# iwa-shi/DC_VIC

Hardware: AMD Instinct MI355X
Metric: images/sec encode+decode @256x256 q=0 (higher is better)
Workload: dtype f32

## Files before the change

dc_vic_amd/csrc/conv.hip:

```cpp
#include "conv_common.h"

template <int MT, int NT, int WM, int WN, bool UPS>
__global__ __launch_bounds__(NTHREADS, (MT * NT >= 8) ? 2 : ((MT * NT >= 4) ? 3 : 4)) void conv_mfma_kernel(const ConvKArgs K) {
    constexpr int TC = WM * MT * 32;
    constexpr int P = WN * NT * 32;
    extern __shared__ __attribute__((aligned(16))) float smem[];
    float* Xs = smem;
    float* Ws = smem + ((K.CPS * KC * K.plane + 3) & ~3);

    const int tid = threadIdx.x;
    const int lane = tid & 63;
    const int wave = tid >> 6;
    const int wm = wave / WN, wn = wave % WN;
    const int lane_k = lane >> 5, lane_j = lane & 31;

    int b;
    {
        const int orig = blockIdx.x, nb = K.nblocks;
        const int q = nb / NXCD, r = nb % NXCD, x = orig % NXCD;
        b = (x < r ? x * (q + 1) : r * (q + 1) + (x - r) * q) + orig / NXCD;
    }
    const int cotile = b % K.n_cotiles; b /= K.n_cotiles;
    const int tile_x = b % K.tiles_x; b /= K.tiles_x;
    const int tile_y = b % K.tiles_y; b /= K.tiles_y;
// ... 277 lines not shown

extern "C" size_t dcvic_conv_packed_bytes(const dcvic_conv_desc* d) {
    if (!d || d->cfg < 0 || d->cfg > 3) return 0;
    return (size_t)n_cotiles_of(d) * n_chunks_of(d) * d->T * KC * cfg_TC(d->cfg) * sizeof(float);
}

extern "C" int dcvic_conv_pack_f32(const dcvic_conv_desc* d, const float* w, float* packed, void* stream) {
    DCVIC_CHECK_ARG(d && w && packed, "conv_pack: null pointer");
    DCVIC_CHECK_ARG(d->cfg >= 0 && d->cfg <= 3, "conv_pack: bad cfg %d", d->cfg);
    const int TC = cfg_TC(d->cfg);
    const long long total = (long long)n_cotiles_of(d) * n_chunks_of(d) * d->T * KC * TC;
    PackTaps taps;
    for (int t = 0; t < DCVIC_MAX_TAPS; ++t) { taps.ky[t] = t < d->T ? d->tap_ky[t] : 0; taps.kx[t] = t < d->T ? d->tap_kx[t] : 0; }
    conv_pack_kernel<<<dcvic_cdiv(total, 256), 256, 0, (hipStream_t)stream>>>(w, packed, d->Cin, d->Cout, d->T, d->KH, d->KW,
                                                                        d->transposed_weight, TC, n_chunks_of(d), total, taps);
    hipError_t e = hipGetLastError();
    if (e != hipSuccess) { dcvic_set_error("conv_pack: %s", hipGetErrorString(e)); return DCVIC_ELAUNCH; }
    return DCVIC_OK;
}

template <int MT, int NT, int WM, int WN>
static int launch_variant(const ConvKArgs& K, bool ups, size_t lds, hipStream_t st) {
    static std::atomic<unsigned> attr_mask{0};
    auto k0 = conv_mfma_kernel<MT, NT, WM, WN, false>;
    auto k1 = conv_mfma_kernel<MT, NT, WM, WN, true>;
    if (DcvicAttrOnce once_{attr_mask}) {
        hipFuncSetAttribute(reinterpret_cast<const void*>(k0), hipFuncAttributeMaxDynamicSharedMemorySize, 160 * 1024);
        hipFuncSetAttribute(reinterpret_cast<const void*>(k1), hipFuncAttributeMaxDynamicSharedMemorySize, 160 * 1024);
    }
    if (ups) k1<<<K.nblocks, NTHREADS, lds, st>>>(K);
    else k0<<<K.nblocks, NTHREADS, lds, st>>>(K);
    DCVIC_CHECK_LAUNCH("conv2d");
    return DCVIC_OK;
}

static void init_num_cu() {
    g_num_cu = dcvic_num_cu();
    if (!g_tuning_init) {
        g_tuning_init = 1;
        const char* e = getenv("DCVIC_CONV_DMA");
        if (e && e[0] == '0') g_use_dma = 0;
        e = getenv("DCVIC_CONV_ASYNC");
        if (e && e[0] == '0') g_use_async = 0;
        e = getenv("DCVIC_CONV_ASYNC16");
        if (e && e[0] == '0') g_use_async16 = 0;
        e = getenv("DCVIC_CONV_ASYNC_FILL");
        if (e && atoi(e) > 0) g_async_fill = atoi(e);
        e = getenv("DCVIC_CONV_ASYNC_FILL256");
        if (e && atoi(e) > 0) g_async_fill256 = atoi(e);
    }
}

extern "C" int dcvic_conv_last_variant(void) { return g_last_variant; }

extern "C" int dcvic_conv_set_tuning(int use_dma, int use_async, int async_fill) {
    init_num_cu();
    if (use_dma >= 0) g_use_dma = use_dma != 0;
    if (use_async >= 0) { g_use_async = use_async != 0; g_use_async16 = use_async != 2; }
    if (async_fill > 0) g_async_fill = async_fill;
    return DCVIC_OK;
}

extern "C" int dcvic_conv_select_class(const dcvic_conv_desc* d, int N, int Hout, int Wout) {
    if (!d || N <= 0 || Hout <= 0 || Wout <= 0) return DCVIC_EINVAL;
    init_num_cu();
    int best_cls = choose_class(d->Cout);
    double best = -1.0;
#ifdef DCVIC_CONV_EXPERIMENTS
    if (const char* e = getenv("DCVIC_FORCE_CLS")) return atoi(e);
#endif
    for (int cls = 0; cls < 4; ++cls)
        for (int pi = 0; pi < kClassNP[cls]; ++pi) {
            const double sc = variant_score(cls, kClassP[cls][pi], d->Cout, N, Hout, Wout, d->upsample, g_num_cu);
            if (sc > best + 1e-9) { best = sc; best_cls = cls; }
        }
    return best_cls;
}

int dcvic_conv_check_io(const DcvicConvRules& r, const void* weights, const dcvic_conv_io* io, ConvKArgs* K) {
    const char* nm = r.name;
    DCVIC_CHECK_ARG(io && io->out && weights && r.Cin > 0 && r.Cout > 0, "%s: null pointer", nm);
    DCVIC_CHECK_ARG(io->n_src >= 1 && io->n_src <= r.max_src, "%s: n_src %d (1..%d)", nm, io->n_src, r.max_src);
    DCVIC_CHECK_ARG(io->N > 0 && io->H > 0 && io->W > 0 && io->Hout > 0 && io->Wout > 0, "%s: bad sizes", nm);
    auto vec16 = [&](const void* p, long long bs) { return !r.vec16 || ((reinterpret_cast<uintptr_t>(p) & 15) == 0 && (bs & 3) == 0); };
    int csum = 0;
    for (int i = 0; i < io->n_src; ++i) {
        const dcvic_src& s = io->src[i];
        DCVIC_CHECK_ARG(s.ptr && s.C > 0 && s.C % r.src_cmul == 0, "%s: source %d empty or not a multiple of %d channels", nm, i, r.src_cmul);
        DCVIC_CHECK_ARG(s.batch_stride >= (long long)s.C * io->H * io->W, "%s: source %d batch stride too small", nm, i);
        DCVIC_CHECK_ARG(vec16(s.ptr, s.batch_stride), "%s: source %d must be a 16-byte aligned view", nm, i);
        csum += s.C;
    }
    DCVIC_CHECK_ARG(csum == r.Cin, "%s: sources carry %d channels, layer expects %d", nm, csum, r.Cin);
    if (r.out_geom == DCVIC_OUT_SCATTER) {
        DCVIC_CHECK_ARG(io->osy >= 1 && io->osx >= 1 && io->ooy >= 0 && io->oox >= 0, "%s: bad output scatter", nm);
        DCVIC_CHECK_ARG((io->Hout - 1) * io->osy + io->ooy < io->Hfull && (io->Wout - 1) * io->osx + io->oox < io->Wfull,
                        "%s: output scatter exceeds the output plane", nm);
    } else {
        const int f = r.out_geom == DCVIC_OUT_X2 ? 2 : 1;
        DCVIC_CHECK_ARG(io->Hout == f * io->H && io->Wout == f * io->W && io->Hfull == io->Hout && io->Wfull == io->Wout && io->osy == 1 &&
                        io->osx == 1 && io->ooy == 0 && io->oox == 0, "%s: output must be the %d x %d plane", nm, f * io->H, f * io->W);
    }
    DCVIC_CHECK_ARG(!r.max_plane || ((long long)io->H * io->W < r.max_plane &&
                                     (r.out_geom != DCVIC_OUT_SCATTER || (long long)io->Hfull * io->Wfull < r.max_plane)),
                    "%s: plane too large", nm);
    const long long out_min = (long long)r.Cout * io->Hfull * io->Wfull;
// ... 161 lines not shown
```

dc_vic_amd/csrc/conv_common.h:

```cpp
#pragma once
#include "common.h"

typedef float f32x16 __attribute__((ext_vector_type(16)));

#define KC 8
#define MAXSLOT 6
#define NTHREADS 256
#define NXCD 8

struct ConvKArgs {
    int Cin, Cout, T, stride;
    int N, H, W, Hout, Wout, Hfull, Wfull, osy, osx, ooy, oox;
    const float* src[DCVIC_MAX_SRC];
    int srcC[DCVIC_MAX_SRC];
    long long src_bs[DCVIC_MAX_SRC];
    float* out;
    long long out_bs;
    const float* bias;
    int act;
    const float* res;
    long long res_bs;
    const float* affs;
    const float* afft;
    long long aff_bs;
// ... 34 lines not shown
#pragma unroll
            for (int r = 0; r < B; ++r) bv[r] = 0.f;
        }
        if constexpr (RES) {
#pragma unroll
            for (int r = 0; r < B; ++r) rv[r] = rp[(long long)min(co_of(r0 + r), cmax) * HWo];
        }
        if constexpr (AFF) {
#pragma unroll
            for (int r = 0; r < B; ++r) { const int c = min(co_of(r0 + r), cmax); sv[r] = K.affs[ab + c]; tv[r] = K.afft[ab + c]; }
        }
#pragma unroll
        for (int r = 0; r < B; ++r) {
            v[r] = accv[r0 + r];
            if (K.bias) v[r] += bv[r];
            v[r] = dcvic_act(v[r], K.act);
            if constexpr (RES) v[r] += rv[r];
            if constexpr (AFF) v[r] = v[r] * (1.f + sv[r]) + tv[r];
        }
#pragma unroll
        for (int r = 0; r < B; ++r) {
            const int co = co_of(r0 + r);
            if (co <= cmax) op[(long long)co * HWo] = v[r];
        }
    }
}

template <class F>
__device__ __forceinline__ void dcvic_epilogue_dispatch(const ConvKArgs& K, F&& f) {
    if (K.res) {
        if (K.affs) f(std::true_type{}, std::true_type{}); else f(std::true_type{}, std::false_type{});
    } else {
        if (K.affs) f(std::false_type{}, std::true_type{}); else f(std::false_type{}, std::false_type{});
    }
}

enum { DCVIC_OUT_SCATTER, DCVIC_OUT_SAME, DCVIC_OUT_X2 };
struct DcvicConvRules {
    const char* name;
    int Cin, Cout;
    int max_src;
    int src_cmul;
    bool vec16;
    int out_geom;
    bool affine;
    bool init;
    long long max_plane;
};

int dcvic_conv_check_io(const DcvicConvRules& r, const void* weights, const dcvic_conv_io* io, ConvKArgs* K);
int dcvic_conv_tiles(const char* name, ConvKArgs* K, int kc, int co, int th, int tw);
int dcvic_persistent_grid(long long nblocks);

int dcvic_try_conv3x3_dma(const ConvKArgs& K, int n_src, bool upsample, int cls, hipStream_t st, int* variant_out);

int dcvic_try_conv_async(const ConvKArgs& K, int cls, int P, hipStream_t st);

int dcvic_try_conv1x1_dma(const ConvKArgs& K, int n_src, bool upsample, int cls, int min_blocks, hipStream_t st);

int dcvic_try_conv_async16(const ConvKArgs& K, int cls, int P, hipStream_t st);
```

dc_vic_amd/csrc/wino44.hip:

```cpp
#include "conv_common.h"

#ifndef DCVIC_W44_DBG
#define DCVIC_W44_DBG 0
#endif

typedef __attribute__((address_space(3))) void* lds_ptr_t;
typedef float f32x2 __attribute__((ext_vector_type(2)));
typedef float f32x4 __attribute__((ext_vector_type(4)));

__device__ float dcvic_w44_zero[16];

#define F4_TH 16
#define F4_TW 32
#define F4_PW 40
#define F4_PROWS 18
#define F4_PLANE 720
#define F4_KC 8
#define F4_SEGS 1440
#define F4_XSLOTS 6
#define F4_XS 6144
#define F4_US 18432
#define F4_VS 9216
#define F4_CO 64
#define F4_THREADS 256
#define F4_OFF_V (2 * F4_XS)
#define F4_OFF_BIAS (F4_OFF_V + 2 * F4_VS)
#define F4_LDS_FLOATS (F4_OFF_BIAS + 2 * F4_CO)

__host__ __device__ constexpr int f4_pos(int a, int b) { return (b >= 1 && b <= 4) ? a * 4 + (b - 1) : 24 + 2 * a + (b == 5 ? 1 : 0); }

__device__ __forceinline__ double f4_u(const float* g, int a, int b) {
    const double G[6][3] = {{64.0 / 81.0, 0.0, 0.0},
                            {-128.0 / 243.0, -32.0 / 81.0, -8.0 / 27.0}, {-128.0 / 243.0, 32.0 / 81.0, -8.0 / 27.0},
                            {32.0 / 243.0, 16.0 / 81.0, 8.0 / 27.0}, {32.0 / 243.0, -16.0 / 81.0, 8.0 / 27.0},
                            {0.0, 0.0, 1.0}};
    double s = 0.0;
#pragma unroll
    for (int r = 0; r < 3; ++r)
#pragma unroll
        for (int c = 0; c < 3; ++c) s += G[a][r] * (double)g[r * 3 + c] * G[b][c];
    return s;
}

__global__ void wino44_pack_kernel(const float* __restrict__ w, float* __restrict__ wp, int Cin, int Cout, int n_chunks, long long total) {
    const long long i = (long long)blockIdx.x * blockDim.x + threadIdx.x;
    if (i >= total) return;
    long long r = i;
    const int slot = r & 3; r >>= 2;
    const int m = r & 15; r >>= 4;
    const int k = r & 3; r >>= 2;
    const int cg = r & 3; r >>= 2;
    const int pg = (int)(r % 9); r /= 9;
    const int ks = (int)(r & 1); r >>= 1;
    const int chunk = (int)(r % n_chunks);
    const int cotile = (int)(r / n_chunks);
    const int idx = pg * 4 + slot;
    int a, b;
    if (idx < 24) { a = idx >> 2; b = (idx & 3) + 1; } else { a = (idx - 24) >> 1; b = ((idx - 24) & 1) ? 5 : 0; }
    const int co = cotile * F4_CO + cg * 16 + m, ci = chunk * F4_KC + 4 * ks + k;
    float v = 0.f;
    if (co < Cout && ci < Cin) v = (float)f4_u(w + ((long long)co * Cin + ci) * 9, a, b);
    wp[i] = v;
}

#define F4_BT_QUARTER(Q, X0, X1, X2, X3, X4, X5, T)                                               \
    do {                                                                                           \
        if constexpr ((Q) == 0) {                                                                  \
            T[0] = __builtin_fmaf(-2.25f, X2, X4);                           \
            T[1] = __builtin_fmaf(-2.25f, X1, X3);                           \
            T[2] = __builtin_fmaf(-0.5625f, X2, X4);                        \
        } else if constexpr ((Q) == 1) {                                                           \
            T[3] = __builtin_fmaf(-0.5625f, X1, X3);                        \
            T[4] = __builtin_fmaf(-2.8125f, X2, X4);                            \
            T[5] = __builtin_fmaf(-2.8125f, X3, X5);                            \
        } else if constexpr ((Q) == 2) {                                                           \
            T[6] = __builtin_fmaf(1.265625f, X0, T[4]);                                    \
            T[7] = __builtin_fmaf(1.265625f, X1, T[5]);                                    \
            T[8] = __builtin_fmaf(0.75f, T[1], T[0]);                                      \
        } else {                                                                                   \
            X2 = __builtin_fmaf(-0.75f, T[1], T[0]);                                       \
            X3 = __builtin_fmaf(1.5f, T[3], T[2]);                                         \
            X4 = __builtin_fmaf(-1.5f, T[3], T[2]);                                        \
            X0 = T[6]; X1 = T[8]; X5 = T[7];                                                       \
        }                                                                                          \
    } while (0)

__device__ __forceinline__ void f4_at(float m0, float m1, float m2, float m3, float m4, float m5, float& y0, float& y1, float& y2, float& y3) {
    const float s12 = m1 + m2, d12 = m1 - m2, s34 = m3 + m4, d34 = m3 - m4;
    y0 = (m0 + s12) + s34;
    y1 = __builtin_fmaf(1.5f, d34, 0.75f * d12);
    y2 = __builtin_fmaf(2.25f, s34, 0.5625f * s12);
    y3 = __builtin_fmaf(3.375f, d34, __builtin_fmaf(0.421875f, d12, m5));
}

__global__ __launch_bounds__(F4_THREADS, 1) void conv3x3_wino44_kernel(const ConvKArgs K) {
    extern __shared__ __attribute__((aligned(16))) float smem[];
    const int tid = threadIdx.x;
    const int lane = tid & 63;
    const int wave = __builtin_amdgcn_readfirstlane(tid >> 6);

    const long long HW = (long long)K.H * K.W;
    const int S = K.n_chunks;
    const long long x_stride = (long long)F4_KC * HW;

    int xe;
    const int J = (int)gridDim.x / NXCD;
    int first;
    {
        const int nb = K.nblocks, q = nb / NXCD, r = nb % NXCD, x = (int)blockIdx.x % NXCD;
        const int xs = x < r ? x * (q + 1) : r * (q + 1) + (x - r) * q;
        xe = xs + (x < r ? q + 1 : q);
        first = xs + (int)blockIdx.x / NXCD;
// ... 93 lines not shown
        if constexpr (q == 3) de[a] = f32x2{dl[a], dr[a]};
    };
    auto t_store = [&](auto i_, unsigned vaddr) {
        constexpr int i = decltype(i_)::value;
        if constexpr (i < 6) {
            const f32x4 v = dm[i];
            asm volatile("ds_write_b128 %0, %1 offset:%2" :: "v"(vaddr), "v"(v), "n"(i * 2048) : "memory");
        } else {
            constexpr int a = i - 6;
            const f32x2 v = de[a];
            asm volatile("ds_write_b64 %0, %1 offset:%2" :: "v"(vaddr), "v"(v), "n"((6 + a / 2) * 2048 + 8 * (a & 1)) : "memory");
        }
    };
    f32x4 uA[2][9];
    f32x4 opB[3][2];
    auto u_load = [&](auto ks_, auto pg_, const float* slab) {
        constexpr int ks = decltype(ks_)::value, pg = decltype(pg_)::value;
        f32x4& dst = uA[ks][pg];
        const float* base = slab + (ks * 9 + pg) * 1024;
        const unsigned vo = u_voff;
        asm volatile("global_load_dwordx4 %0, %1, %2" : "=v"(dst) : "v"(vo), "s"(base) : "memory");
    };
    auto op_load = [&](auto G_, unsigned va) {
        constexpr int G = decltype(G_)::value, set = G % 3, ks = G / 9, pg = G % 9;
        f32x4 &b0 = opB[set][0], &b1 = opB[set][1];
        asm volatile("ds_read_b128 %0, %1 offset:%2" : "=v"(b0) : "v"(va), "n"(ks * 18432 + 1024 * (2 * pg)));
        asm volatile("ds_read_b128 %0, %1 offset:%2" : "=v"(b1) : "v"(va), "n"(ks * 18432 + 1024 * (2 * pg + 1)));
    };
    auto dma_x = [&](auto s_, int buf) {
        constexpr int sl = decltype(s_)::value;
        __builtin_amdgcn_global_load_lds(reinterpret_cast<const float4*>(xp[sl]), (lds_ptr_t)(smem + buf * F4_XS + (wave * 64 + sl * F4_THREADS) * 4), 16, 0, 0);
    };
    auto x_advance = [&]() __attribute__((always_inline)) {
        if (++x_next == S) {
            x_next = 0;
            x_b += J;
            if (x_b < xe) x_setup(x_b);
        } else {
            x_left -= F4_KC;
            if (x_left > 0) {
#pragma unroll
                for (int sl = 0; sl < F4_XSLOTS; ++sl) xp[sl] += poff[sl] >= 0 ? x_stride : 0ll;
            } else {
                x_rebase(x_next * F4_KC);
            }
        }
    };

    float* const sbias = smem + F4_OFF_BIAS;
    const int e_n = lane & 15, lq = lane >> 4;
    const float neg_slope = K.act == DCVIC_ACT_RELU ? 0.f : K.act == DCVIC_ACT_LRELU02 ? 0.2f : 1.f;
    const bool has_bias = K.bias != nullptr, has_res = K.res != nullptr;
    auto tile_epilogue = [&](int cotile, int n, int oy0, int ox0, int par) __attribute__((always_inline)) {
        asm volatile("s_nop 15\n\ts_nop 15" ::: "memory");
        auto A = [&](auto idx_, auto blk_, int r) __attribute__((always_inline)) -> float {
            constexpr int idx = decltype(idx_)::value, blk = decltype(blk_)::value;
            if constexpr (idx < 32) {
                float v;
                const float src = acc[idx][blk][r];
                asm volatile("v_accvgpr_read_b32 %0, %1" : "=v"(v) : "a"(src));
                return v;
            } else return accv[idx - 32][blk][r];
        };
        const int co0 = cotile * F4_CO + cg * 16 + 4 * lq;
        float bv[4];
#pragma unroll
        for (int r = 0; r < 4; ++r) bv[r] = has_bias ? sbias[par * F4_CO + cg * 16 + 4 * lq + r] : 0.f;
        float gs[4] = {0.f, 0.f, 0.f, 0.f}, gq[4] = {0.f, 0.f, 0.f, 0.f};
        dcvic_static_for<0, 2>([&](auto blk_) {
            constexpr int blk = decltype(blk_)::value;
            const int t = blk * 16 + e_n;
            const int oy = oy0 + 4 * (t >> 3), ox = ox0 + 4 * (t & 7);
            const int rows = K.H - oy;
            const bool in_img = ox < K.W && rows > 0;
            const long long pix = (long long)oy * K.W + ox;
#pragma unroll
            for (int r = 0; r < 4; ++r) {
                float tm[4][6];
                dcvic_static_for<0, 6>([&](auto b_) {
                    constexpr int b = decltype(b_)::value;
                    f4_at(A(std::integral_constant<int, f4_pos(0, b)>{}, blk_, r), A(std::integral_constant<int, f4_pos(1, b)>{}, blk_, r),
                          A(std::integral_constant<int, f4_pos(2, b)>{}, blk_, r), A(std::integral_constant<int, f4_pos(3, b)>{}, blk_, r),
                          A(std::integral_constant<int, f4_pos(4, b)>{}, blk_, r), A(std::integral_constant<int, f4_pos(5, b)>{}, blk_, r),
                          tm[0][b], tm[1][b], tm[2][b], tm[3][b]);
                });
                float y[4][4];
#pragma unroll
                for (int i = 0; i < 4; ++i) {
                    f4_at(tm[i][0], tm[i][1], tm[i][2], tm[i][3], tm[i][4], tm[i][5], y[i][0], y[i][1], y[i][2], y[i][3]);
#pragma unroll
                    for (int j = 0; j < 4; ++j) y[i][j] += bv[r];
                }
#pragma unroll
                for (int i = 0; i < 4; ++i)
#pragma unroll
                    for (int j = 0; j < 4; ++j) y[i][j] = y[i][j] > 0.f ? y[i][j] : neg_slope * y[i][j];
                if (in_img && co0 + r < K.Cout) {
                    float* const ob = K.out + (long long)n * K.out_bs + (long long)(co0 + r) * HW + pix;
                    const bool want_gn = K.gn_part != nullptr;
                    if (has_res) {
                        const float* const rb = K.res + (long long)n * K.res_bs + (long long)(co0 + r) * HW + pix;
                        f32x4 rv[4];
#pragma unroll
                        for (int i = 0; i < 4; ++i) rv[i] = *reinterpret_cast<const f32x4*>(rb + (long long)min(i, rows - 1) * K.W);
#pragma unroll
                        for (int i = 0; i < 4; ++i)
#pragma unroll
                            for (int j = 0; j < 4; ++j) y[i][j] += rv[i][j];
                    }
                    if (want_gn) {
#pragma unroll
                        for (int i = 0; i < 4; ++i)
                            if (i < rows) {
#pragma unroll
                                for (int j = 0; j < 4; ++j) { gs[r] += y[i][j]; gq[r] = __builtin_fmaf(y[i][j], y[i][j], gq[r]); }
                            }
                    }
                    if (rows >= 4) {
#pragma unroll
                        for (int i = 0; i < 4; ++i) *reinterpret_cast<f32x4*>(ob + (long long)i * K.W) = f32x4{y[i][0], y[i][1], y[i][2], y[i][3]};
                    } else {
#pragma unroll
                        for (int i = 0; i < 3; ++i)
                            if (i < rows) *reinterpret_cast<f32x4*>(ob + (long long)i * K.W) = f32x4{y[i][0], y[i][1], y[i][2], y[i][3]};
                    }
                }
            }
        });
        if (K.gn_part) {
#pragma unroll
            for (int r = 0; r < 4; ++r) {
#pragma unroll
                for (int o = 1; o < 16; o <<= 1) { gs[r] += __shfl_xor(gs[r], o, 64); gq[r] += __shfl_xor(gq[r], o, 64); }
            }
            if (e_n == 0) {
                const int pt = (oy0 / F4_TH) * K.tiles_x + ox0 / F4_TW;
                const int npt = K.tiles_x * K.tiles_y;
#pragma unroll
                for (int r = 0; r < 4; ++r)
                    if (co0 + r < K.Cout)
                        *reinterpret_cast<f32x2*>(K.gn_part + (((long long)n * K.Cout + co0 + r) * npt + pt) * 2) = f32x2{gs[r], gq[r]};
            }
        }
    };
    auto stage_bias = [&](int b, int par) __attribute__((always_inline)) {
        if (tid < F4_CO) sbias[par * F4_CO + tid] = has_bias ? K.bias[min(cotile_of(b) * F4_CO + tid, K.Cout - 1)] : 0.f;
    };

    int c_b = first, c_par = 0;
    int c_cotile, c_n, c_oy0, c_ox0;
    decode(first, c_cotile, c_n, c_oy0, c_ox0);
    stage_bias(first, 0);
    dcvic_static_for<0, F4_XSLOTS>([&](auto s_) { dma_x(s_, 0); });
    x_advance();
    if (total > 1) {
        dcvic_static_for<0, F4_XSLOTS>([&](auto s_) { dma_x(s_, 1); });
        x_advance();
    }
    dcvic_static_for<0, 9>([&](auto pg_) { u_load(std::integral_constant<int, 0>{}, pg_, wp_cur); });
    asm volatile("s_waitcnt vmcnt(0)" ::: "memory");
    __syncthreads();
    F4_FENCE();
    dcvic_static_for<0, 6>([&](auto r_) { t_load(r_, t_src); });
    F4_WAIT_LDS();
    dcvic_static_for<0, 6>([&](auto c_) { dcvic_static_for<0, 4>([&](auto q_) { t_col(c_, q_); }); });
    dcvic_static_for<0, 6>([&](auto a_) { dcvic_static_for<0, 4>([&](auto q_) { t_row(a_, q_); }); });
    dcvic_static_for<0, 12>([&](auto i_) { t_store(i_, t_dst); });
    F4_WAIT_LDS();
    __syncthreads();
    F4_FENCE();
    op_load(std::integral_constant<int, 0>{}, op_v);

    auto run_stage = [&](int s) __attribute__((always_inline)) {
        const int cur = s & 1, nxt = cur ^ 1;
        const unsigned va = op_v + (unsigned)(cur * F4_VS * 4);
        const unsigned xaddr = t_src + (unsigned)(nxt * F4_XS * 4);
        const unsigned vaddr = t_dst + (unsigned)(nxt * F4_VS * 4);
        dcvic_static_for<0, 18>([&](auto G_) {
            constexpr int G = decltype(G_)::value, ks = G / 9, pg = G % 9, set = G % 3;
            if constexpr (G < 17) {
// ... 18 lines not shown
                    if constexpr (pg < 8) asm volatile("v_mfma_f32_16x16x4_f32 %0, %1, %2, %0" : "+a"(acc[pg * 4 + ps][blk]) : "v"(a_), "v"(b_));
                    else asm volatile("v_mfma_f32_16x16x4_f32 %0, %1, %2, %0" : "+v"(accv[ps][blk]) : "v"(a_), "v"(b_));
                }
                F4_FENCE();
                constexpr int sl = 8 * G + q;
                constexpr int h = sl % 72;
                if constexpr (!(DCVIC_W44_DBG & 4) && (h & 3) == 1 && h < 12) dma_x(std::integral_constant<int, 3 * ks + h / 4>{}, cur);
                if constexpr (!(DCVIC_W44_DBG & 4) && (h & 3) == 1 && h >= 12 && h < 48) {
                    if constexpr (ks == 0) u_load(std::integral_constant<int, 1>{}, std::integral_constant<int, (h / 4 - 3)>{}, wp_cur);
                    else u_load(std::integral_constant<int, 0>{}, std::integral_constant<int, (h / 4 - 3)>{}, wp_nxt);
                }
                if constexpr (!(DCVIC_W44_DBG & 2)) {
                    if constexpr (sl < 12 && (sl & 3) >= 2) t_load(std::integral_constant<int, ((sl / 4) * 2 + (sl & 1))>{}, xaddr);
                    if constexpr (sl >= 16 && sl < 64 && (sl & 1) == 0)
                        t_col(std::integral_constant<int, (((sl - 16) / 2) / 4)>{}, std::integral_constant<int, (((sl - 16) / 2) % 4)>{});
                    if constexpr (sl >= 72 && sl < 120 && (sl & 1) == 0)
                        t_row(std::integral_constant<int, (((sl - 72) / 2) / 4)>{}, std::integral_constant<int, (((sl - 72) / 2) % 4)>{});
                    if constexpr (sl >= 120 && sl < 132) t_store(std::integral_constant<int, sl - 120>{}, vaddr);
                }
                F4_FENCE();
            });
        });
        F4_FENCE();
    };
    {
        int s = 0;
        for (int t = 0; t < ntile; ++t) {
#pragma unroll
            for (int i = 0; i < 32; ++i)
#pragma unroll
                for (int j = 0; j < 2; ++j) acc[i][j] = f32x4{0.f, 0.f, 0.f, 0.f};
#pragma unroll
            for (int i = 0; i < 4; ++i)
#pragma unroll
                for (int j = 0; j < 2; ++j) accv[i][j] = f32x4{0.f, 0.f, 0.f, 0.f};
            for (int c = 0; c < S; ++c, ++s) {
                run_stage(s);
                if (s + 2 < total) x_advance();
                wp_cur = wp_nxt;
                if (s + 2 < total) u_advance();
            }
            if constexpr (!(DCVIC_W44_DBG & 16)) tile_epilogue(c_cotile, c_n, c_oy0, c_ox0, c_par);
            c_b += J; c_par ^= 1;
            if (c_b < xe) {
                decode(c_b, c_cotile, c_n, c_oy0, c_ox0);
                stage_bias(c_b, c_par);
            }
        }
    }
#undef F4_FENCE
#undef F4_WAIT_LDS
}

extern "C" size_t dcvic_wino44_packed_bytes(int Cin, int Cout) {
    if (Cin <= 0 || Cout <= 0) return 0;
    return (size_t)((Cout + F4_CO - 1) / F4_CO) * ((Cin + F4_KC - 1) / F4_KC) * F4_US * sizeof(float);
}

extern "C" int dcvic_wino44_pack_f32(const float* w, float* packed, int Cin, int Cout, void* stream) {
    DCVIC_CHECK_ARG(w && packed && Cin > 0 && Cout > 0, "wino44_pack: bad argument");
    const int n_chunks = (Cin + F4_KC - 1) / F4_KC;
    const long long total = (long long)((Cout + F4_CO - 1) / F4_CO) * n_chunks * F4_US;
    wino44_pack_kernel<<<dcvic_cdiv(total, 256), 256, 0, (hipStream_t)stream>>>(w, packed, Cin, Cout, n_chunks, total);
    DCVIC_CHECK_LAUNCH("wino44_pack");
    return DCVIC_OK;
}

extern "C" int dcvic_wino44_stats_tiles(int H, int W) { return H > 0 && W > 0 ? ((H + F4_TH - 1) / F4_TH) * ((W + F4_TW - 1) / F4_TW) : 0; }

static int wino44_launch(int Cin, int Cout, const float* packed, const dcvic_conv_io* io, float* gn_part, void* stream);

extern "C" int dcvic_conv3x3_wino44_f32(int Cin, int Cout, const float* packed, const dcvic_conv_io* io, void* stream) {
    return wino44_launch(Cin, Cout, packed, io, nullptr, stream);
}

extern "C" int dcvic_conv3x3_wino44_stats_f32(int Cin, int Cout, const float* packed, const dcvic_conv_io* io, float* gn_part, void* stream) {
    DCVIC_CHECK_ARG(gn_part, "conv3x3_wino44_stats: null statistics buffer");
    return wino44_launch(Cin, Cout, packed, io, gn_part, stream);
}

static int wino44_launch(int Cin, int Cout, const float* packed, const dcvic_conv_io* io, float* gn_part, void* stream) {
    const DcvicConvRules rules = {"conv3x3_wino44", Cin, Cout, DCVIC_MAX_SRC, F4_KC, true, DCVIC_OUT_SAME, false, false, 1ll << 28};
    ConvKArgs K;
    if (const int rc = dcvic_conv_check_io(rules, packed, io, &K)) return rc;
    DCVIC_CHECK_ARG((io->W & 3) == 0, "conv3x3_wino44: width must be a multiple of 4");
    DCVIC_CHECK_ARG(io->act == DCVIC_ACT_NONE || io->act == DCVIC_ACT_RELU || io->act == DCVIC_ACT_LRELU02,
                    "conv3x3_wino44: activation %d not supported (none / ReLU / LeakyReLU(0.2) only)", io->act);
    K.gn_part = gn_part;
    if (const int rc = dcvic_conv_tiles("conv3x3_wino44", &K, F4_KC, F4_CO, F4_TH, F4_TW)) return rc;
    static std::atomic<unsigned> attr_mask{0};
    if (DcvicAttrOnce once_{attr_mask})
        hipFuncSetAttribute(reinterpret_cast<const void*>(conv3x3_wino44_kernel), hipFuncAttributeMaxDynamicSharedMemorySize, 160 * 1024);
    conv3x3_wino44_kernel<<<dcvic_persistent_grid(K.nblocks), F4_THREADS, F4_LDS_FLOATS * sizeof(float), (hipStream_t)stream>>>(K);
    DCVIC_CHECK_LAUNCH("conv3x3_wino44");
    return DCVIC_OK;
}
```

Before: 205.5.

## Add 128-output-channel Winograd F(4,3) kernel with half-height tiles for wide convs

Adds a second Winograd F(4x4,3x3) kernel that covers 128 output channels per block and processes each 16x32 spatial tile as two 8-row halves, for layers whose Cout is a multiple of 128. Weight packing gains a wide layout that interleaves two 16-channel groups per wave. The goal is to reuse each transformed input tile across twice as many output channels, halving input-transform and input-load work per output. The cost is heavy register pressure, with accumulators held in AGPRs, occupancy limited to one block per CU, and a more complex pipelined schedule. Group-norm statistics are now accumulated across both halves.

```diff
diff --git a/dc_vic_amd/csrc/conv.hip b/dc_vic_amd/csrc/conv.hip
--- a/dc_vic_amd/csrc/conv.hip
+++ b/dc_vic_amd/csrc/conv.hip
@@ -353,6 +353,7 @@
 }
 
 extern "C" int dcvic_conv_last_variant(void) { return g_last_variant; }
+void dcvic_conv_note_variant(int variant) { g_last_variant = variant; }
 
 extern "C" int dcvic_conv_set_tuning(int use_dma, int use_async, int async_fill) {
     init_num_cu();
diff --git a/dc_vic_amd/csrc/conv_common.h b/dc_vic_amd/csrc/conv_common.h
--- a/dc_vic_amd/csrc/conv_common.h
+++ b/dc_vic_amd/csrc/conv_common.h
@@ -110,6 +110,8 @@
 int dcvic_conv_tiles(const char* name, ConvKArgs* K, int kc, int co, int th, int tw);
 int dcvic_persistent_grid(long long nblocks);
 
+void dcvic_conv_note_variant(int variant);
+
 int dcvic_try_conv3x3_dma(const ConvKArgs& K, int n_src, bool upsample, int cls, hipStream_t st, int* variant_out);
 
 int dcvic_try_conv_async(const ConvKArgs& K, int cls, int P, hipStream_t st);
diff --git a/dc_vic_amd/csrc/wino44.hip b/dc_vic_amd/csrc/wino44.hip
--- a/dc_vic_amd/csrc/wino44.hip
+++ b/dc_vic_amd/csrc/wino44.hip
@@ -26,6 +26,17 @@
 #define F4_OFF_V (2 * F4_XS)
 #define F4_OFF_BIAS (F4_OFF_V + 2 * F4_VS)
 #define F4_LDS_FLOATS (F4_OFF_BIAS + 2 * F4_CO)
+#define F8_CO 128
+#define F8_TH 8
+#define F8_PLANE 400
+#define F8_SEGS 800
+#define F8_XSLOTS 4
+#define F8_XS 4096
+#define F8_US 36864
+#define F8_VS 4608
+#define F8_OFF_V (2 * F8_XS)
+#define F8_OFF_BIAS (F8_OFF_V + 2 * F8_VS)
+#define F8_LDS_FLOATS (F8_OFF_BIAS + 2 * F8_CO)
 
 __host__ __device__ constexpr int f4_pos(int a, int b) { return (b >= 1 && b <= 4) ? a * 4 + (b - 1) : 24 + 2 * a + (b == 5 ? 1 : 0); }
 
@@ -42,13 +53,15 @@
     return s;
 }
 
-__global__ void wino44_pack_kernel(const float* __restrict__ w, float* __restrict__ wp, int Cin, int Cout, int n_chunks, long long total) {
+__global__ void wino44_pack_kernel(const float* __restrict__ w, float* __restrict__ wp, int Cin, int Cout, int n_chunks, long long total, int wide) {
     const long long i = (long long)blockIdx.x * blockDim.x + threadIdx.x;
     if (i >= total) return;
     long long r = i;
     const int slot = r & 3; r >>= 2;
     const int m = r & 15; r >>= 4;
     const int k = r & 3; r >>= 2;
+    int cgrp = 0;
+    if (wide) { cgrp = r & 1; r >>= 1; }
     const int cg = r & 3; r >>= 2;
     const int pg = (int)(r % 9); r /= 9;
     const int ks = (int)(r & 1); r >>= 1;
@@ -57,7 +70,7 @@
     const int idx = pg * 4 + slot;
     int a, b;
     if (idx < 24) { a = idx >> 2; b = (idx & 3) + 1; } else { a = (idx - 24) >> 1; b = ((idx - 24) & 1) ? 5 : 0; }
-    const int co = cotile * F4_CO + cg * 16 + m, ci = chunk * F4_KC + 4 * ks + k;
+    const int co = wide ? cotile * F8_CO + cg * 32 + cgrp * 16 + m : cotile * F4_CO + cg * 16 + m, ci = chunk * F4_KC + 4 * ks + k;
     float v = 0.f;
     if (co < Cout && ci < Cin) v = (float)f4_u(w + ((long long)co * Cin + ci) * 9, a, b);
     wp[i] = v;
@@ -455,6 +468,395 @@
 #undef F4_WAIT_LDS
 }
 
+#define F8_BT_HALF(H, STEP, L0, L1, L2, L3, L4, T)                                                 \
+    do {                                                                                           \
+        if constexpr ((H) == 0 && (STEP) == 0) {                                                   \
+            T[0] = __builtin_fmaf(-2.25f, L2, L4);                                         \
+            T[1] = __builtin_fmaf(-2.25f, L1, L3);                                         \
+            T[2] = __builtin_fmaf(-2.8125f, L2, L4);                                               \
+        } else if constexpr ((H) == 0) {                                                           \
+            L0 = __builtin_fmaf(1.265625f, L0, T[2]);                                      \
+            L1 = __builtin_fmaf(0.75f, T[1], T[0]);                                        \
+            L2 = __builtin_fmaf(-0.75f, T[1], T[0]);                                       \
+        } else if constexpr ((STEP) == 0) {                                                        \
+            T[0] = __builtin_fmaf(-0.5625f, L1, L3);                        \
+            T[1] = __builtin_fmaf(-0.5625f, L0, L2);                        \
+            T[2] = __builtin_fmaf(-2.8125f, L2, L4);                            \
+        } else {                                                                                   \
+            L2 = __builtin_fmaf(1.265625f, L0, T[2]);                                      \
+            L0 = __builtin_fmaf(1.5f, T[1], T[0]);                                         \
+            L1 = __builtin_fmaf(-1.5f, T[1], T[0]);                                        \
+        }                                                                                          \
+    } while (0)
+
+__global__ __launch_bounds__(F4_THREADS, 1) void conv3x3_wino44_kernel_c128(const ConvKArgs K) {
+    extern __shared__ __attribute__((aligned(16))) float smem[];
+    const int tid = threadIdx.x;
+    const int lane = tid & 63;
+    const int wave = __builtin_amdgcn_readfirstlane(tid >> 6);
+
+    const long long HW = (long long)K.H * K.W;
+    const int S = K.n_chunks;
+    const long long x_stride = (long long)F4_KC * HW;
+
+    int xe;
+    const int J = (int)gridDim.x / NXCD;
+    int first;
+    {
+        const int nb = K.nblocks, q = nb / NXCD, r = nb % NXCD, x = (int)blockIdx.x % NXCD;
+        const int xs = x < r ? x * (q + 1) : r * (q + 1) + (x - r) * q;
+        xe = xs + (x < r ? q + 1 : q);
+        first = xs + (int)blockIdx.x / NXCD;
+    }
+    if (first >= xe) return;
+    const int npass = 2 * ((xe - first + J - 1) / J);
+    const int total = npass * S;
+    const int n_ptiles = K.nblocks / K.n_cotiles;
+    auto decode = [&](int b, int h, int& cotile, int& n, int& oy0, int& ox0) __attribute__((always_inline)) {
+        cotile = b / n_ptiles; b -= cotile * n_ptiles;
+        const int tile_x = b % K.tiles_x; b /= K.tiles_x;
+        const int tile_y = b % K.tiles_y; b /= K.tiles_y;
+        n = b; oy0 = tile_y * F4_TH + h * F8_TH; ox0 = tile_x * F4_TW;
+    };
+    auto cotile_of = [&](int b) __attribute__((always_inline)) { return b / n_ptiles; };
+
+    const float* xp[F8_XSLOTS];
+    int poff[F8_XSLOTS];
+    int x_left = 0, x_n = 0, x_b = first, x_h = 0, x_next = 0;
+    auto x_rebase = [&](int c) __attribute__((always_inline)) {
+        int si = 0;
+        if (c >= K.srcC[0]) { c -= K.srcC[0]; si = 1; if (c >= K.srcC[1]) { c -= K.srcC[1]; si = 2; } }
+        const float* base = K.src[si] + (long long)x_n * K.src_bs[si] + (long long)c * HW;
+#pragma unroll
+        for (int s = 0; s < F8_XSLOTS; ++s) xp[s] = poff[s] >= 0 ? base + poff[s] : dcvic_w44_zero;
+        x_left = K.srcC[si] - c;
+    };
+    auto x_setup = [&](int b, int h) __attribute__((always_inline)) {
+        int cot, oy0, ox0;
+        decode(b, h, cot, x_n, oy0, ox0);
+#pragma unroll
+        for (int s = 0; s < F8_XSLOTS; ++s) {
+            const int e = tid + s * F4_THREADS;
+            int o = -1;
+            if (e < F8_SEGS) {
+                const int k = e / 100, r = e - k * 100;
+                const int py = r / 10, seg = r - py * 10;
+                const int iy = oy0 - 1 + py, ix = ox0 - 4 + 4 * seg;
+                if (iy >= 0 && iy < K.H && ix >= 0 && ix < K.W) o = (int)(k * HW) + iy * K.W + ix;
+            }
+            poff[s] = o;
+        }
+        x_rebase(0);
+    };
+    x_setup(first, 0);
+    const int cg = wave;
+    const unsigned u_voff = 16u * (unsigned)(cg * 128 + lane);
+    const float* wp_cur;
+    const float* wp_nxt;
+    int u_b = first, u_h = 0, u_next = 0;
+    auto u_setup = [&](int b) __attribute__((always_inline)) { wp_nxt = K.wp + (long long)cotile_of(b) * S * (long long)F8_US; };
+    u_setup(first);
+    wp_cur = wp_nxt;
+    auto u_advance = [&]() __attribute__((always_inline)) {
+        if (++u_next == S) {
+            u_next = 0;
+            if (u_h == 0) { u_h = 1; u_setup(u_b); }
+            else { u_h = 0; u_b += J; if (u_b < xe) u_setup(u_b); }
+        } else {
+            wp_nxt += F8_US;
+        }
+    };
+    u_advance();
+
+    const unsigned op_v = 4u * (unsigned)(F8_OFF_V + lane * 4);
+
+    f32x4 acc[32][2];
+    f32x4 accv[4][2];
+    float gs[2][4], gq[2][4];
+
+#define F4_FENCE() __builtin_amdgcn_sched_barrier(0)
+#define F4_WAIT_LDS() do { asm volatile("s_waitcnt lgkmcnt(0)" ::: "memory"); F4_FENCE(); } while (0)
+    f32x4 uA[9][2];
+    f32x4 opB[3];
+    auto u_load = [&](auto ks_, auto pg_, auto g_, const float* slab) {
+        constexpr int ks = decltype(ks_)::value, pg = decltype(pg_)::value, g = decltype(g_)::value;
+        f32x4& dst = uA[pg][g];
+        const float* base = slab + (ks * 9 + pg) * 2048;
+        const unsigned vo = u_voff;
+        asm volatile("global_load_dwordx4 %0, %1, %2 offset:%3" : "=v"(dst) : "v"(vo), "s"(base), "n"(g * 1024) : "memory");
+    };
+    auto op_load = [&](auto G_, unsigned va) {
+        constexpr int G = decltype(G_)::value, set = G % 3, ks = G / 9, pg = G % 9;
+        f32x4& b0 = opB[set];
+        asm volatile("ds_read_b128 %0, %1 offset:%2" : "=v"(b0) : "v"(va), "n"(ks * 9216 + 1024 * pg));
+    };
+    auto dma_x = [&](auto s_, int buf) {
+        constexpr int sl = decltype(s_)::value;
+        __builtin_amdgcn_global_load_lds(reinterpret_cast<const float4*>(xp[sl]), (lds_ptr_t)(smem + buf * F8_XS + (wave * 64 + sl * F4_THREADS) * 4), 16, 0, 0);
+    };
+    auto x_advance = [&]() __attribute__((always_inline)) {
+        if (++x_next == S) {
+            x_next = 0;
+            if (x_h == 0) { x_h = 1; x_setup(x_b, 1); }
+            else { x_h = 0; x_b += J; if (x_b < xe) x_setup(x_b, 0); }
+        } else {
+            x_left -= F4_KC;
+            if (x_left > 0) {
+#pragma unroll
+                for (int sl = 0; sl < F8_XSLOTS; ++sl) xp[sl] += poff[sl] >= 0 ? x_stride : 0ll;
+            } else {
+                x_rebase(x_next * F4_KC);
+            }
+        }
+    };
+
+    float* const sbias = smem + F8_OFF_BIAS;
+    const int e_n = lane & 15, lq = lane >> 4;
+    const float neg_slope = K.act == DCVIC_ACT_RELU ? 0.f : K.act == DCVIC_ACT_LRELU02 ? 0.2f : 1.f;
+    const bool has_bias = K.bias != nullptr, has_res = K.res != nullptr;
+    auto tile_epilogue = [&](int cotile, int n, int oy0, int ox0, int par, int h) __attribute__((always_inline)) {
+        asm volatile("s_nop 15\n\ts_nop 15" ::: "memory");
+        auto A = [&](auto idx_, auto g_, int r) __attribute__((always_inline)) -> float {
+            constexpr int idx = decltype(idx_)::value, g = decltype(g_)::value;
+            if constexpr (idx < 32) {
+                float v;
+                const float src = acc[idx][g][r];
+                asm volatile("v_accvgpr_read_b32 %0, %1" : "=v"(v) : "a"(src));
+                return v;
+            } else return accv[idx - 32][g][r];
+        };
+        const int oy = oy0 + 4 * (e_n >> 3), ox = ox0 + 4 * (e_n & 7);
+        const int rows = K.H - oy;
+        const bool in_img = ox < K.W && rows > 0;
+        const long long pix = (long long)oy * K.W + ox;
+        dcvic_static_for<0, 2>([&](auto g_) {
+            constexpr int g = decltype(g_)::value;
+            const int co0 = cotile * F8_CO + cg * 32 + g * 16 + 4 * lq;
+            float bv[4];
+#pragma unroll
+            for (int r = 0; r < 4; ++r) bv[r] = has_bias ? sbias[par * F8_CO + cg * 32 + g * 16 + 4 * lq + r] : 0.f;
+#pragma unroll
+            for (int r = 0; r < 4; ++r) {
+                if (h == 0) { gs[g][r] = 0.f; gq[g][r] = 0.f; }
+                float tm[4][6];
+                dcvic_static_for<0, 6>([&](auto b_) {
+                    constexpr int b = decltype(b_)::value;
+                    f4_at(A(std::integral_constant<int, f4_pos(0, b)>{}, g_, r), A(std::integral_constant<int, f4_pos(1, b)>{}, g_, r),
+                          A(std::integral_constant<int, f4_pos(2, b)>{}, g_, r), A(std::integral_constant<int, f4_pos(3, b)>{}, g_, r),
+                          A(std::integral_constant<int, f4_pos(4, b)>{}, g_, r), A(std::integral_constant<int, f4_pos(5, b)>{}, g_, r),
+                          tm[0][b], tm[1][b], tm[2][b], tm[3][b]);
+                });
+                float y[4][4];
+#pragma unroll
+                for (int i = 0; i < 4; ++i) {
+                    f4_at(tm[i][0], tm[i][1], tm[i][2], tm[i][3], tm[i][4], tm[i][5], y[i][0], y[i][1], y[i][2], y[i][3]);
+#pragma unroll
+                    for (int j = 0; j < 4; ++j) y[i][j] += bv[r];
+                }
+#pragma unroll
+                for (int i = 0; i < 4; ++i)
+#pragma unroll
+                    for (int j = 0; j < 4; ++j) y[i][j] = y[i][j] > 0.f ? y[i][j] : neg_slope * y[i][j];
+                if (in_img) {
+                    float* const ob = K.out + (long long)n * K.out_bs + (long long)(co0 + r) * HW + pix;
+                    const bool want_gn = K.gn_part != nullptr;
+                    if (has_res) {
+                        const float* const rb = K.res + (long long)n * K.res_bs + (long long)(co0 + r) * HW + pix;
+                        f32x4 rv[4];
+#pragma unroll
+                        for (int i = 0; i < 4; ++i) rv[i] = *reinterpret_cast<const f32x4*>(rb + (long long)min(i, rows - 1) * K.W);
+#pragma unroll
+                        for (int i = 0; i < 4; ++i)
+#pragma unroll
+                            for (int j = 0; j < 4; ++j) y[i][j] += rv[i][j];
+                    }
+                    if (want_gn) {
+#pragma unroll
+                        for (int i = 0; i < 4; ++i)
+                            if (i < rows) {
+#pragma unroll
+                                for (int j = 0; j < 4; ++j) { gs[g][r] += y[i][j]; gq[g][r] = __builtin_fmaf(y[i][j], y[i][j], gq[g][r]); }
+                            }
+                    }
+                    if (rows >= 4) {
+#pragma unroll
+                        for (int i = 0; i < 4; ++i) *reinterpret_cast<f32x4*>(ob + (long long)i * K.W) = f32x4{y[i][0], y[i][1], y[i][2], y[i][3]};
+                    } else {
+#pragma unroll
+                        for (int i = 0; i < 3; ++i)
+                            if (i < rows) *reinterpret_cast<f32x4*>(ob + (long long)i * K.W) = f32x4{y[i][0], y[i][1], y[i][2], y[i][3]};
+                    }
+                }
+            }
+        });
+        if (K.gn_part && h == 1) {
+            const int pt = ((oy0 - F8_TH) / F4_TH) * K.tiles_x + ox0 / F4_TW;
+            const int npt = K.tiles_x * K.tiles_y;
+#pragma unroll
+            for (int g = 0; g < 2; ++g)
+#pragma unroll
+                for (int r = 0; r < 4; ++r) {
+                    float a = gs[g][r], b = gq[g][r];
+#pragma unroll
+                    for (int o = 1; o < 16; o <<= 1) { a += __shfl_xor(a, o, 64); b += __shfl_xor(b, o, 64); }
+                    const int co = cotile * F8_CO + cg * 32 + g * 16 + 4 * lq + r;
+                    if (e_n == 0) *reinterpret_cast<f32x2*>(K.gn_part + (((long long)n * K.Cout + co) * npt + pt) * 2) = f32x2{a, b};
+                }
+        }
+    };
+    auto stage_bias = [&](int b, int par) __attribute__((always_inline)) {
+        if (tid < F8_CO) sbias[par * F8_CO + tid] = has_bias ? K.bias[cotile_of(b) * F8_CO + tid] : 0.f;
+    };
+
+    auto run_all = [&](auto half_) __attribute__((always_inline)) {
+        constexpr int HALF = decltype(half_)::value;
+        const int t_p = tid & 127, t_k = t_p >> 4, t_n = t_p & 15, t_ty = t_n >> 3, t_tx = t_n & 7;
+        const unsigned t_src = 4u * (unsigned)(t_k * F8_PLANE + (4 * t_ty + HALF) * F4_PW + 4 * t_tx + 3);
+        const unsigned t_dst = 4u * (unsigned)(F8_OFF_V + (t_k >> 2) * 2304 + ((t_k & 3) * 16 + t_n) * 4);
+        float dl[5], dr[5];
+        f32x4 dm[5];
+        f32x2 de[3];
+        float tt[9];
+        auto t_load = [&](auto r_, unsigned xaddr) {
+            constexpr int r = decltype(r_)::value;
+            float &l = dl[r], &rr = dr[r];
+            f32x4 &m = dm[r];
+            asm volatile("ds_read_b32 %0, %1 offset:%2" : "=v"(l) : "v"(xaddr), "n"(4 * (r * F4_PW)));
+            asm volatile("ds_read_b128 %0, %1 offset:%2" : "=v"(m) : "v"(xaddr), "n"(4 * (r * F4_PW + 1)));
+            asm volatile("ds_read_b32 %0, %1 offset:%2" : "=v"(rr) : "v"(xaddr), "n"(4 * (r * F4_PW + 5)));
+        };
+        auto t_col = [&](auto c_, auto st_) {
+            constexpr int c = decltype(c_)::value, st = decltype(st_)::value;
+            if constexpr (c == 0) F8_BT_HALF(HALF, st, dl[0], dl[1], dl[2], dl[3], dl[4], tt);
+            else if constexpr (c == 5) F8_BT_HALF(HALF, st, dr[0], dr[1], dr[2], dr[3], dr[4], tt);
+            else { constexpr int e = c == 0 || c == 5 ? 0 : c - 1; F8_BT_HALF(HALF, st, dm[0][e], dm[1][e], dm[2][e], dm[3][e], dm[4][e], tt); }
+        };
+        auto t_row = [&](auto a_, auto q_) {
+            constexpr int a = decltype(a_)::value, q = decltype(q_)::value;
+            F4_BT_QUARTER(q, dl[a], dm[a][0], dm[a][1], dm[a][2], dm[a][3], dr[a], tt);
+            if constexpr (q == 3) de[a] = f32x2{dl[a], dr[a]};
+        };
+        auto t_store = [&](auto i_, unsigned vaddr) {
+            constexpr int i = decltype(i_)::value, a = 3 * HALF + i % 3;
+            if constexpr (i < 3) {
+                const f32x4 v = dm[i];
+                asm volatile("ds_write_b128 %0, %1 offset:%2" :: "v"(vaddr), "v"(v), "n"(a * 1024) : "memory");
+            } else {
+                const f32x2 v = de[i - 3];
+                asm volatile("ds_write_b64 %0, %1 offset:%2" :: "v"(vaddr), "v"(v), "n"((6 + a / 2) * 1024 + 8 * (a & 1)) : "memory");
+            }
+        };
+
+        int c_b = first, c_h = 0, c_par = 0;
+        int c_cotile, c_n, c_oy0, c_ox0;
+        decode(first, 0, c_cotile, c_n, c_oy0, c_ox0);
+        stage_bias(first, 0);
+        dcvic_static_for<0, F8_XSLOTS>([&](auto s_) { dma_x(s_, 0); });
+        x_advance();
+        if (total > 1) {
+            dcvic_static_for<0, F8_XSLOTS>([&](auto s_) { dma_x(s_, 1); });
+            x_advance();
+        }
+        dcvic_static_for<0, 9>([&](auto pg_) {
+            u_load(std::integral_constant<int, 0>{}, pg_, std::integral_constant<int, 0>{}, wp_cur);
+            u_load(std::integral_constant<int, 0>{}, pg_, std::integral_constant<int, 1>{}, wp_cur);
+        });
+        asm volatile("s_waitcnt vmcnt(0)" ::: "memory");
+        __syncthreads();
+        F4_FENCE();
+        dcvic_static_for<0, 5>([&](auto r_) { t_load(r_, t_src); });
+        F4_WAIT_LDS();
+        dcvic_static_for<0, 6>([&](auto c_) { dcvic_static_for<0, 2>([&](auto st_) { t_col(c_, st_); }); });
+        dcvic_static_for<0, 3>([&](auto a_) { dcvic_static_for<0, 4>([&](auto q_) { t_row(a_, q_); }); });
+        dcvic_static_for<0, 6>([&](auto i_) { t_store(i_, t_dst); });
+        F4_WAIT_LDS();
+        __syncthreads();
+        F4_FENCE();
+        op_load(std::integral_constant<int, 0>{}, op_v);
+
+        auto run_stage = [&](int s, bool last) __attribute__((always_inline)) {
+            const int cur = s & 1, nxt = cur ^ 1;
+            const unsigned va = op_v + (unsigned)(cur * F8_VS * 4);
+            const unsigned xaddr = t_src + (unsigned)(nxt * F8_XS * 4);
+            const unsigned vaddr = t_dst + (unsigned)(nxt * F8_VS * 4);
+            dcvic_static_for<0, 18>([&](auto G_) {
+                constexpr int G = decltype(G_)::value, ks = G / 9, pg = G % 9, set = G % 3;
+                if constexpr (G < 17) {
+                    if constexpr (!(DCVIC_W44_DBG & 8)) {
+                        if constexpr (pg == 0) asm volatile("s_waitcnt vmcnt(16) lgkmcnt(0)" ::: "memory");
+                        else asm volatile("s_waitcnt vmcnt(18) lgkmcnt(0)" ::: "memory");
+                        F4_FENCE();
+                        op_load(std::integral_constant<int, G + 1>{}, va);
+                    }
+                } else {
+                    if constexpr (DCVIC_W44_DBG & 64) asm volatile("s_waitcnt lgkmcnt(0)" ::: "memory");
+                    else asm volatile("s_waitcnt vmcnt(15) lgkmcnt(0)" ::: "memory");
+                    if constexpr (!(DCVIC_W44_DBG & 1)) __builtin_amdgcn_s_barrier();
+                    F4_FENCE();
+                    if constexpr (!(DCVIC_W44_DBG & 8)) op_load(std::integral_constant<int, 0>{}, op_v + (unsigned)(nxt * F8_VS * 4));
+                }
+                F4_FENCE();
+                dcvic_static_for<0, 8>([&](auto q_) {
+                    constexpr int q = decltype(q_)::value, g = q >> 2, ps = q & 3;
+                    if constexpr (!(DCVIC_W44_DBG & 32)) {
+                        const float a_ = uA[pg][g][ps], b_ = opB[set][ps];
+                        if constexpr (pg < 8) asm volatile("v_mfma_f32_16x16x4_f32 %0, %1, %2, %0" : "+a"(acc[pg * 4 + ps][g]) : "v"(a_), "v"(b_));
+                        else asm volatile("v_mfma_f32_16x16x4_f32 %0, %1, %2, %0" : "+v"(accv[ps][g]) : "v"(a_), "v"(b_));
+                    }
+                    F4_FENCE();
+                    constexpr int sl = 8 * G + q;
+                    if constexpr (!(DCVIC_W44_DBG & 4)) {
+                        if constexpr (pg == 0 && (q == 1 || q == 5)) dma_x(std::integral_constant<int, 2 * ks + q / 4>{}, cur);
+                        if constexpr ((q & 3) == 3) {
+                            if constexpr (ks == 0) u_load(std::integral_constant<int, 1>{}, std::integral_constant<int, pg>{}, std::integral_constant<int, g>{}, wp_cur);
+                            else u_load(std::integral_constant<int, 0>{}, std::integral_constant<int, pg>{}, std::integral_constant<int, g>{}, wp_nxt);
+                        }
+                    }
+                    if constexpr (!(DCVIC_W44_DBG & 2)) {
+                        if constexpr (sl < 11 && (sl & 3) >= 2) t_load(std::integral_constant<int, ((sl / 4) * 2 + (sl & 1))>{}, xaddr);
+                        if constexpr (sl >= 16 && sl < 64 && (sl & 3) == 0)
+                            t_col(std::integral_constant<int, (((sl - 16) / 4) / 2)>{}, std::integral_constant<int, (((sl - 16) / 4) % 2)>{});
+                        if constexpr (sl >= 72 && sl < 120 && (sl & 3) == 0)
+                            t_row(std::integral_constant<int, (((sl - 72) / 4) / 4)>{}, std::integral_constant<int, (((sl - 72) / 4) % 4)>{});
+                        if constexpr (sl >= 120 && sl < 126) t_store(std::integral_constant<int, sl - 120>{}, vaddr);
+                    }
+                    F4_FENCE();
+                });
+            });
+            if (last) asm volatile("s_waitcnt vmcnt(0)" ::: "memory");
+            F4_FENCE();
+        };
+        int s = 0;
+        for (int t = 0; t < npass; ++t) {
+#pragma unroll
+            for (int i = 0; i < 32; ++i)
+#pragma unroll
+                for (int j = 0; j < 2; ++j) acc[i][j] = f32x4{0.f, 0.f, 0.f, 0.f};
+#pragma unroll
+            for (int i = 0; i < 4; ++i)
+#pragma unroll
+                for (int j = 0; j < 2; ++j) accv[i][j] = f32x4{0.f, 0.f, 0.f, 0.f};
+            for (int c = 0; c < S; ++c, ++s) {
+                run_stage(s, c == S - 1);
+                if (s + 2 < total) x_advance();
+                wp_cur = wp_nxt;
+                if (s + 2 < total) u_advance();
+            }
+            if constexpr (!(DCVIC_W44_DBG & 16)) tile_epilogue(c_cotile, c_n, c_oy0, c_ox0, c_par, c_h);
+            c_par ^= 1;
+            if (c_h == 0) c_h = 1; else { c_h = 0; c_b += J; }
+            if (c_b < xe) {
+                decode(c_b, c_h, c_cotile, c_n, c_oy0, c_ox0);
+                stage_bias(c_b, c_par);
+            }
+        }
+    };
+    if (wave < 2) run_all(std::integral_constant<int, 0>{});
+    else run_all(std::integral_constant<int, 1>{});
+#undef F4_FENCE
+#undef F4_WAIT_LDS
+}
+
 extern "C" size_t dcvic_wino44_packed_bytes(int Cin, int Cout) {
     if (Cin <= 0 || Cout <= 0) return 0;
     return (size_t)((Cout + F4_CO - 1) / F4_CO) * ((Cin + F4_KC - 1) / F4_KC) * F4_US * sizeof(float);
@@ -464,7 +866,7 @@
     DCVIC_CHECK_ARG(w && packed && Cin > 0 && Cout > 0, "wino44_pack: bad argument");
     const int n_chunks = (Cin + F4_KC - 1) / F4_KC;
     const long long total = (long long)((Cout + F4_CO - 1) / F4_CO) * n_chunks * F4_US;
-    wino44_pack_kernel<<<dcvic_cdiv(total, 256), 256, 0, (hipStream_t)stream>>>(w, packed, Cin, Cout, n_chunks, total);
+    wino44_pack_kernel<<<dcvic_cdiv(total, 256), 256, 0, (hipStream_t)stream>>>(w, packed, Cin, Cout, n_chunks, total, Cout % F8_CO == 0);
     DCVIC_CHECK_LAUNCH("wino44_pack");
     return DCVIC_OK;
 }
@@ -490,11 +892,21 @@
     DCVIC_CHECK_ARG(io->act == DCVIC_ACT_NONE || io->act == DCVIC_ACT_RELU || io->act == DCVIC_ACT_LRELU02,
                     "conv3x3_wino44: activation %d not supported (none / ReLU / LeakyReLU(0.2) only)", io->act);
     K.gn_part = gn_part;
-    if (const int rc = dcvic_conv_tiles("conv3x3_wino44", &K, F4_KC, F4_CO, F4_TH, F4_TW)) return rc;
+    const bool wide = Cout % F8_CO == 0;
+    if (const int rc = dcvic_conv_tiles("conv3x3_wino44", &K, F4_KC, wide ? F8_CO : F4_CO, F4_TH, F4_TW)) return rc;
     static std::atomic<unsigned> attr_mask{0};
-    if (DcvicAttrOnce once_{attr_mask})
+    if (DcvicAttrOnce once_{attr_mask}) {
         hipFuncSetAttribute(reinterpret_cast<const void*>(conv3x3_wino44_kernel), hipFuncAttributeMaxDynamicSharedMemorySize, 160 * 1024);
+        hipFuncSetAttribute(reinterpret_cast<const void*>(conv3x3_wino44_kernel_c128), hipFuncAttributeMaxDynamicSharedMemorySize, 160 * 1024);
+    }
+    if (wide) {
+        conv3x3_wino44_kernel_c128<<<dcvic_persistent_grid(K.nblocks), F4_THREADS, F8_LDS_FLOATS * sizeof(float), (hipStream_t)stream>>>(K);
+        DCVIC_CHECK_LAUNCH("conv3x3_wino44");
+        dcvic_conv_note_variant(9106);
+        return DCVIC_OK;
+    }
     conv3x3_wino44_kernel<<<dcvic_persistent_grid(K.nblocks), F4_THREADS, F4_LDS_FLOATS * sizeof(float), (hipStream_t)stream>>>(K);
     DCVIC_CHECK_LAUNCH("conv3x3_wino44");
+    dcvic_conv_note_variant(9104);
     return DCVIC_OK;
 }
```

Measured after the change: 210.4 (median of 5 runs). 2.4% higher.

## Prefetch residual tiles in Winograd epilogue with manual vmcnt pipelining

Applied to the files above, without the earlier changes.

The residual loads in the F(4,3) Winograd epilogue are now issued ahead of use through inline global_load_dwordx4, kept four iterations deep in a ring of register slots. Explicit s_waitcnt vmcnt values replace the load-then-use pattern so residual latency overlaps the output transforms and stores. Out-of-range lanes read from a zero buffer instead of branching. This raises register pressure and depends on hand-counted vmcnt values that are only exact for full tiles; partial tiles fall back to a more conservative wait.

```diff
diff --git a/dc_vic_amd/csrc/wino44.hip b/dc_vic_amd/csrc/wino44.hip
--- a/dc_vic_amd/csrc/wino44.hip
+++ b/dc_vic_amd/csrc/wino44.hip
@@ -26,6 +26,7 @@
 #define F4_OFF_V (2 * F4_XS)
 #define F4_OFF_BIAS (F4_OFF_V + 2 * F4_VS)
 #define F4_LDS_FLOATS (F4_OFF_BIAS + 2 * F4_CO)
+#define F4_RD 4
 
 __host__ __device__ constexpr int f4_pos(int a, int b) { return (b >= 1 && b <= 4) ? a * 4 + (b - 1) : 24 + 2 * a + (b == 5 ? 1 : 0); }
 
@@ -257,6 +258,28 @@
     const float neg_slope = K.act == DCVIC_ACT_RELU ? 0.f : K.act == DCVIC_ACT_LRELU02 ? 0.2f : 1.f;
     const bool has_bias = K.bias != nullptr, has_res = K.res != nullptr;
     auto tile_epilogue = [&](int cotile, int n, int oy0, int ox0, int par) __attribute__((always_inline)) {
+        const int co0 = cotile * F4_CO + cg * 16 + 4 * lq;
+        f32x4 rv[F4_RD][4];
+        const float* const rbase = has_res ? K.res + (long long)n * K.res_bs + (long long)co0 * HW : nullptr;
+        auto res_issue = [&](auto it_) __attribute__((always_inline)) {
+            constexpr int it = decltype(it_)::value, blk = it >> 2, r = it & 3, sl = it % F4_RD;
+            const int t = blk * 16 + e_n;
+            const int oy = oy0 + 4 * (t >> 3), ox = ox0 + 4 * (t & 7);
+            const int rows = K.H - oy;
+            const bool ok = !(DCVIC_W44_DBG & 128) && ox < K.W && rows > 0 && co0 + r < K.Cout;
+            const float* const rb = rbase + (long long)r * HW + ((long long)oy * K.W + ox);
+#pragma unroll
+            for (int i = 0; i < 4; ++i) {
+                const float* const p = ok ? rb + (long long)min(i, rows - 1) * K.W : dcvic_w44_zero;
+                f32x4& dst = rv[sl][i];
+                asm volatile("global_load_dwordx4 %0, %1, off" : "=v"(dst) : "v"(p) : "memory");
+            }
+        };
+        bool full = false;
+        if (has_res) {
+            full = !(DCVIC_W44_DBG & 256) && oy0 + F4_TH <= K.H && ox0 + F4_TW <= K.W && __all(co0 + 3 < K.Cout);
+            dcvic_static_for<0, F4_RD>([&](auto it_) { res_issue(it_); });
+        }
         asm volatile("s_nop 15\n\ts_nop 15" ::: "memory");
         auto A = [&](auto idx_, auto blk_, int r) __attribute__((always_inline)) -> float {
             constexpr int idx = decltype(idx_)::value, blk = decltype(blk_)::value;
@@ -267,7 +290,6 @@
                 return v;
             } else return accv[idx - 32][blk][r];
         };
-        const int co0 = cotile * F4_CO + cg * 16 + 4 * lq;
         float bv[4];
 #pragma unroll
         for (int r = 0; r < 4; ++r) bv[r] = has_bias ? sbias[par * F4_CO + cg * 16 + 4 * lq + r] : 0.f;
@@ -279,8 +301,8 @@
             const int rows = K.H - oy;
             const bool in_img = ox < K.W && rows > 0;
             const long long pix = (long long)oy * K.W + ox;
-#pragma unroll
-            for (int r = 0; r < 4; ++r) {
+            dcvic_static_for<0, 4>([&](auto r_) {
+                constexpr int r = decltype(r_)::value, it = 4 * blk + r;
                 float tm[4][6];
                 dcvic_static_for<0, 6>([&](auto b_) {
                     constexpr int b = decltype(b_)::value;
@@ -300,19 +322,25 @@
                 for (int i = 0; i < 4; ++i)
 #pragma unroll
                     for (int j = 0; j < 4; ++j) y[i][j] = y[i][j] > 0.f ? y[i][j] : neg_slope * y[i][j];
+                if (has_res) {
+                    constexpr int sl = it % F4_RD;
+                    constexpr int n_ld = 4 * ((it + F4_RD - 1 < 7 ? it + F4_RD - 1 : 7) - it), n_st = 4 * (it < F4_RD ? it : F4_RD);
+                    if constexpr (!(DCVIC_W44_DBG & 128)) {
+                        if (full) asm volatile("s_waitcnt vmcnt(%0)" :: "n"(n_ld + n_st) : "memory");
+                        else asm volatile("s_waitcnt vmcnt(%0)" :: "n"(n_ld) : "memory");
+                    }
+                    asm volatile("" : "+v"(rv[sl][0]), "+v"(rv[sl][1]), "+v"(rv[sl][2]), "+v"(rv[sl][3]) :: "memory");
+                    if (in_img && co0 + r < K.Cout) {
+#pragma unroll
+                        for (int i = 0; i < 4; ++i)
+#pragma unroll
+                            for (int j = 0; j < 4; ++j) y[i][j] += rv[sl][i][j];
+                    }
+                    if constexpr (it + F4_RD < 8) res_issue(std::integral_constant<int, it + F4_RD>{});
+                }
                 if (in_img && co0 + r < K.Cout) {
                     float* const ob = K.out + (long long)n * K.out_bs + (long long)(co0 + r) * HW + pix;
                     const bool want_gn = K.gn_part != nullptr;
-                    if (has_res) {
-                        const float* const rb = K.res + (long long)n * K.res_bs + (long long)(co0 + r) * HW + pix;
-                        f32x4 rv[4];
-#pragma unroll
-                        for (int i = 0; i < 4; ++i) rv[i] = *reinterpret_cast<const f32x4*>(rb + (long long)min(i, rows - 1) * K.W);
-#pragma unroll
-                        for (int i = 0; i < 4; ++i)
-#pragma unroll
-                            for (int j = 0; j < 4; ++j) y[i][j] += rv[i][j];
-                    }
                     if (want_gn) {
 #pragma unroll
                         for (int i = 0; i < 4; ++i)
@@ -321,7 +349,9 @@
                                 for (int j = 0; j < 4; ++j) { gs[r] += y[i][j]; gq[r] = __builtin_fmaf(y[i][j], y[i][j], gq[r]); }
                             }
                     }
-                    if (rows >= 4) {
+                    if constexpr (DCVIC_W44_DBG & 256) {
+                        asm volatile("" :: "v"(y[0][0]), "v"(y[1][1]), "v"(y[2][2]), "v"(y[3][3]), "v"(ob));
+                    } else if (rows >= 4) {
 #pragma unroll
                         for (int i = 0; i < 4; ++i) *reinterpret_cast<f32x4*>(ob + (long long)i * K.W) = f32x4{y[i][0], y[i][1], y[i][2], y[i][3]};
                     } else {
@@ -330,7 +360,7 @@
                             if (i < rows) *reinterpret_cast<f32x4*>(ob + (long long)i * K.W) = f32x4{y[i][0], y[i][1], y[i][2], y[i][3]};
                     }
                 }
-            }
+            });
         });
         if (K.gn_part) {
 #pragma unroll
```

Result: no change. 205.4 before, 206.5 after, median of 5 (+0.5%).
